# ZJU-FAST-Lab/uneven_planner

Measured on AMD Instinct MI355X. Metric: MINCO traj-opts/sec (batch), higher is better.
Workload: dtype f64

## Files before the change

uneven_planner_amd/csrc/solver_program.hpp:

```cpp
#pragma once
#include "terrain_dev.hpp"
#include "trajectory_dev.hpp"
#include "uph_common.hpp"

namespace uph {

#ifndef UPH_GRID_FROM_MEM
#define UPH_GRID_FROM_MEM 1
#endif
#ifndef UPH_PHASE_MASK
#define UPH_PHASE_MASK 15
#endif
#ifndef UPH_STATE_PROBE
#define UPH_STATE_PROBE(st) do { } while (0)
#endif
#ifndef UPH_SCALING_WB
#define UPH_SCALING_WB 8
#endif
#ifndef UPH_SC_XB
#define UPH_SC_XB 9
#endif
#ifndef UPH_SC_YB
#define UPH_SC_YB 14
#endif
#ifndef UPH_SC_WLO
#define UPH_SC_WLO 2
#endif
#ifndef UPH_SC_WHI
#define UPH_SC_WHI 3
#endif

template <class WG, class SR = double>
struct Solver {
    WG& wg;
    const GridDev& grid;
    const OptParams& P;
    const BatchDev& bd;
    const TrajDesc& td;
    int Nxy, Nyaw, n, S, K, mem, CH, CHP, recd;
    int CHS;
    int* rtag;
    double *x, *xp, *g, *gp, *d, *cxy, *cyaw, *Gxy, *Gyaw, *gamxy, *gamyaw, *bt, *rec, *wtab, *ttab, *pf, *hd;
    double* ab;
    int* abn;
    static constexpr int AB_DOUBLES = 4;
    UPH_HD void tally(int k, bool yes) {
#if defined(__HIP_DEVICE_COMPILE__)
        if (yes && wg.wave == 0) abn[k] = abn[k] + 1;
#else
        if (yes) abn[k]++;
#endif
    }
    double *dual, *res, *scl, *hist;
    int hrow, hnp;
    const double *Wr_xy, *Wr_yaw;
    double rho, scale_fx, Txy, Tyaw, last_jerk, last_gd;
    long long hist_reads;
    long long cyc[16];
    long long t_last_eval_end;
    long long* sub_t = nullptr;
    int evals, bidx, trace_n;
    float inv_k1;
    double ec_irho, ec_step, ec_invK, ec_iTyaw, ec_omega, ec_omega_h;

    static constexpr int REC_FIELDS = 12;
    static UPH_HD size_t ldsDoubles(int Nxy, int Nyaw, int n, int CH, int mem, int K) {
        size_t recd = (size_t)REC_FIELDS * (CH + 1) + (CH + 1) / 2;
        const size_t nvec = 2 * (Nxy + 5) + (Nyaw + 5);
        const size_t knd = (size_t)knotBufDoubles(Nxy + 1, 4) + knotBufDoubles(Nyaw + 1, 2), adj = (size_t)knotBufDoubles(Nxy, 4) + knotBufDoubles(Nyaw, 2) + nvec;
        recd = recd < knd ? knd : recd;
        recd = recd < adj ? adj : recd;
        recd = recd < (size_t)mem ? (size_t)mem : recd;
        const size_t td_ = (size_t)Nxy + K + 2;
        return (size_t)5 * n + (nvec < td_ ? td_ : nvec) + 2 * (12 * Nxy + 6 * Nyaw) + recd + (size_t)6 * (K + 1) + THOMAS_DOUBLES + MAX_PAST + 8 + 18 + AB_DOUBLES;
    }

    UPH_HD Solver(WG& w, const GridDev& gr, const OptParams& p, const BatchDev& b, int bi, double* lds)
        : wg(w), grid(gr), P(p), bd(b), td(b.desc[bi]) {
        bidx = bi;
        Nxy = td.Nxy; Nyaw = td.Nyaw; n = td.n; S = td.S; K = P.int_K; mem = P.mem_size;
        inv_k1 = 1.0f / (float)(K + 1);
        CH = wg.size(); CHP = CH + 1; recd = REC_FIELDS * CHP + (CH + 1) / 2;
        CHS = CH;
#if !defined(UPH_ALIGNED_CHUNKS) || UPH_ALIGNED_CHUNKS
        {
            const int ppc = CH / (K + 1);
            if (ppc >= 1 && (Nxy + ppc - 1) / ppc == (S + CH - 1) / CH) CHS = ppc * (K + 1);
        }
#endif
        double* q = lds;
        x = q; q += n; g = q; q += n; d = q; q += n;
        xp = q; q += n; gp = q; q += n;
        const int nvec = 2 * (Nxy + 5) + (Nyaw + 5);
        bt = q;
        gamxy = q; gamyaw = q + 2 * (Nxy + 5);
        q += nvec < Nxy + K + 2 ? Nxy + K + 2 : nvec;
        cxy = q; q += 12 * Nxy; cyaw = q; q += 6 * Nyaw;
        Gxy = q; q += 12 * Nxy; Gyaw = q; q += 6 * Nyaw;
        wtab = q; q += 6 * (K + 1);
        rec = q;
        {
            size_t rd = (size_t)recd;
            const size_t knd = (size_t)knotBufDoubles(Nxy + 1, 4) + knotBufDoubles(Nyaw + 1, 2), adj = (size_t)knotBufDoubles(Nxy, 4) + knotBufDoubles(Nyaw, 2) + nvec;
            rd = rd < knd ? knd : rd; rd = rd < adj ? adj : rd; rd = rd < (size_t)mem ? (size_t)mem : rd;
            q += rd;
        }
        rtag = (int*)(rec + (size_t)REC_FIELDS * CHP);
        ttab = q; q += THOMAS_DOUBLES;
        pf = q; q += MAX_PAST + 8;
        hd = q; q += 18;
        ab = q; q += AB_DOUBLES;
        abn = (int*)(ab + 1);
        dual = bd.dual + 7 * td.off_s; res = bd.res + 7 * td.off_s; scl = bd.scl + 7 * td.off_s;
        hist = bd.hist + td.off_hist; hrow = histRowDoubles(n); hnp = 64 * histNQ(n);
        Wr_xy = bd.ops[td.op_xy].Wr; Wr_yaw = bd.ops[td.op_yaw].Wr;
        rho = 0; scale_fx = 1.0; Txy = Tyaw = 0; last_jerk = 0; hist_reads = 0; evals = 0; trace_n = 0;
        for (int q = 0; q < 16; q++) cyc[q] = 0;
        t_last_eval_end = 0;
        wg.pfor(18 + THOMAS_DOUBLES, [&](int t) {
            if (t == 0) { ab[0] = 0.0; abn[0] = abn[1] = abn[2] = abn[3] = 0; }
            if (t < 18) hd[t] = t < 6 ? td.init_xy[t] : (t < 12 ? td.end_xy[t - 6] : (t < 15 ? td.init_yaw[t - 12] : td.end_yaw[t - 15]));
            else ttab[t - 18] = bd.thomas[t - 18];
        });
    }

    UPH_HD void tracePush(double v) {
        if (bd.trace != nullptr && trace_n < bd.trace_cap) {
            const int at = trace_n;
            wg.one([&]() { bd.trace[(size_t)bidx * bd.trace_cap + at] = v; });
        }
        trace_n++;
    }

    static UPH_HD int divSmall(int a, int b, float inv) {
        int q = (int)((float)a * inv);
        const int r = a - q * b;
        if (r < 0) q--;
        else if (r >= b) q++;
        return q;
    }
    static UPH_HD int knotCol(int j, int N) { return j == 0 ? 0 : (j == N ? N + 2 : j + 2); }
    UPH_HD double knotPos(const double* xin, int j, int dd) const {
        if (dd < 2) return j == 0 ? hd[dd] : (j == Nxy ? hd[6 + dd] : xin[1 + 2 * (j - 1) + dd]);
        return j == 0 ? hd[12] : (j == Nyaw ? hd[15] : xin[1 + 2 * (Nxy - 1) + (j - 1)]);
    }

    UPH_HD double dot(const double* a, const double* b, int m) {
        double r[1];
        wg.template sum<1>(m, r, [&](int i, double* acc) { acc[0] += a[i] * b[i]; });
        return r[0];
    }
    UPH_HD double absmax(const double* a, int m) {
        return wg.maxv(m, [&](int i) { return fabs(a[i]); });
    }

    template <bool STEP>
    UPH_HD void generate(double* xin, double st) {
        UPH_MARK("generate");
        const long long tsub_start = wg.clock();
        const double tau_ = STEP ? fma(st, d[0], xp[0]) : xin[0];
        const double Ttot = expC2(tau_);
        Txy = wg.bcast(Ttot / (double)Nxy);
        Tyaw = wg.bcast(Ttot / (double)Nyaw);
        ec_iTyaw = wg.bcast(1.0 / Tyaw);
        const double Tx = Txy, Ty = Tyaw;
        double* zxy = rec;
        double* zyaw = rec + knotBufDoubles(Nxy + 1, 4);
        wg.pfor(2 * (Nxy + 1) + (Nyaw + 1), [&](int t) {
            const bool isxy = t < 2 * (Nxy + 1);
            const int j = isxy ? (t >> 1) : t - 2 * (Nxy + 1), dd = isxy ? (t & 1) : 2, N = isxy ? Nxy : Nyaw, os = isxy ? 2 : 1;
            const double T1 = isxy ? Tx : Ty;
            const double* h0 = isxy ? hd + (dd & 1) : hd + 12;
            const double* h1 = isxy ? hd + 6 + (dd & 1) : hd + 15;
            double* z = isxy ? zxy + knotOffJ(j, 4) + (dd & 1) : zyaw + knotOffJ(j, 2);
            if (STEP && t == 0) xin[0] = tau_;
            if (j == 0) { z[0] = T1 * h0[os]; z[os] = T1 * T1 * h0[2 * os]; }
            else if (j == N) { z[0] = T1 * h1[os]; z[os] = T1 * T1 * h1[2 * os]; }
            else {
                double pm, p0, pp;
                if (STEP) {
                    const int ix = isxy ? 1 + 2 * (j - 1) + dd : 1 + 2 * (Nxy - 1) + (j - 1), ws = isxy ? 2 : 1;
                    p0 = fma(st, d[ix], xp[ix]);
                    pm = j == 1 ? h0[0] : fma(st, d[ix - ws], xp[ix - ws]);
                    pp = j == N - 1 ? h1[0] : fma(st, d[ix + ws], xp[ix + ws]);
                    xin[ix] = p0;
                } else { pm = knotPos(xin, j - 1, dd); p0 = knotPos(xin, j, dd); pp = knotPos(xin, j + 1, dd); }
                const double dp = pp - p0, dm = p0 - pm;
                double r0 = 20.0 * (dp - dm), r1 = -15.0 * (dp + dm);
                if (j == 1) { const double v0 = T1 * h0[os], a0 = T1 * T1 * h0[2 * os]; r0 += 8.0 * v0 + a0; r1 += 7.0 * v0 + a0; }
                if (j == N - 1) { const double vN = T1 * h1[os], aN = T1 * T1 * h1[2 * os]; r0 += -8.0 * vN + aN; r1 += 7.0 * vN - aN; }
                z[0] = r0; z[os] = r1;
            }
        });
        const long long tsub1 = wg.clock();
        wg.thomas(ttab, false, zyaw + knotOffJ(1, 2), Nyaw - 1, zxy + knotOffJ(1, 4), Nxy - 1);
        if (sub_t) { sub_t[0] += tsub1 - tsub_start; sub_t[1] += wg.clock() - tsub1; }
    }

    UPH_HD void expand(const double* xin, double jerk_w, double out[3]) {
        UPH_MARK("expand");
        const long long t0 = wg.clock();
        const double Tx = Txy, Ty = Tyaw, itx = wg.bcast(1.0 / Tx), ity = wg.bcast(1.0 / Ty);
        const double* zxy = rec;
        const double* zyaw = rec + knotBufDoubles(Nxy + 1, 4);
        const int np = 2 * Nxy + Nyaw;
        wg.template sum<3>(np + 2, out, [&](int t, double* acc) {
            if (t >= np) { fillTimes(t - np); return; }
            double p0, p1, v0, a0, v1, a1, it_, T1;
            double *oc, *og;
            int os;
            const bool isxy = t < 2 * Nxy;
            if (isxy) {
                const int i = t >> 1, dd = t & 1;
                p0 = knotPos(xin, i, dd); p1 = knotPos(xin, i + 1, dd);
                const double *k0 = zxy + knotOffJ(i, 4) + dd, *k1 = zxy + knotOffJ(i + 1, 4) + dd;
                v0 = k0[0]; a0 = k0[2]; v1 = k1[0]; a1 = k1[2];
                oc = cxy + 12 * i + dd; og = Gxy + 12 * i + dd; os = 2; it_ = itx; T1 = Tx;
            } else {
                const int m = t - 2 * Nxy;
                p0 = knotPos(xin, m, 2); p1 = knotPos(xin, m + 1, 2);
                const double *k0 = zyaw + knotOffJ(m, 2), *k1 = zyaw + knotOffJ(m + 1, 2);
                v0 = k0[0]; a0 = k0[1]; v1 = k1[0]; a1 = k1[1];
                oc = cyaw + 6 * m; og = Gyaw + 6 * m; os = 1; it_ = ity; T1 = Ty;
            }
            const double dl = p1 - p0;
            const double h3 = 10.0 * dl - 6.0 * v0 - 4.0 * v1 - 1.5 * a0 + 0.5 * a1;
            const double h4 = -15.0 * dl + 8.0 * v0 + 7.0 * v1 + 1.5 * a0 - a1;
            const double h5 = 6.0 * dl - 3.0 * v0 - 3.0 * v1 - 0.5 * a0 + 0.5 * a1;
            const double i2 = it_ * it_, i3 = i2 * it_, i4 = i3 * it_, i5 = i4 * it_;
            const double c3 = h3 * i3, c4 = h4 * i4, c5 = h5 * i5;
            oc[0] = p0; oc[os] = v0 * it_; oc[2 * os] = (0.5 * a0) * i2;
            oc[3 * os] = c3; oc[4 * os] = c4; oc[5 * os] = c5;
            const double T2 = T1 * T1, T3 = T2 * T1, T4 = T2 * T2, T5 = T4 * T1;
            og[0] = 0.0; og[os] = 0.0; og[2 * os] = 0.0;
            og[3 * os] = jerk_w * (72.0 * c3 * T1 + 144.0 * c4 * T2 + 240.0 * c5 * T3);
            og[4 * os] = jerk_w * (144.0 * c3 * T2 + 384.0 * c4 * T3 + 720.0 * c5 * T4);
            og[5 * os] = jerk_w * (240.0 * c3 * T3 + 720.0 * c4 * T4 + 1440.0 * c5 * T5);
            const double d33 = c3 * c3, d43 = c4 * c3, d44 = c4 * c4, d53 = c5 * c3, d54 = c5 * c4, d55 = c5 * c5;
            acc[0] += 36.0 * d33 * T1 + 144.0 * d43 * T2 + 192.0 * d44 * T3 + 240.0 * d53 * T3 + 720.0 * d54 * T4 + 720.0 * d55 * T5;
            const double gT = 36.0 * d33 + 288.0 * d43 * T1 + 576.0 * d44 * T2 + 720.0 * d53 * T2 + 2880.0 * d54 * T3 + 3600.0 * d55 * T4;
            acc[1] += isxy ? gT : 0.0;
            acc[2] += isxy ? 0.0 : gT;
        });
        if (sub_t) sub_t[2] += wg.clock() - t0;
    }

    UPH_HD GridDev framedGrid() const {
        if (bd.grid_mem != nullptr && bd.grid_per_traj != 0) return bd.grid_mem[bidx];
        return grid;
    }

    template <class R>
    struct KinT {
        R b0[6], b1[6], b2[6], b3[6];
        R y0[6], y1[6], y2[6];
        R pos[2], vel[2], acc[2], jer[2];
        R yaw, dyaw, d2yaw, cyaw, syaw, v_norm, lon_acc, lat_acc, u, s1;
        R tv[7], tg[7][3];
        R vx, wz, ax, ay, curv_snorm, den, sq;
        R yawn, cw, sw;
        R zx, zy, gs[3], gzx[3], gzy[3];
        int yaw_idx;
    };
    typedef KinT<double> Kin;
    template <class R>
    UPH_HD void terrainValuesOnly(KinT<R>& S_) const {
        R sg;
#if defined(__HIP_DEVICE_COMPILE__) && UPH_GRID_FROM_MEM
        typedef const __attribute__((address_space(4))) unsigned long long* gw_t;
        gw_t T = (gw_t)(const void*)(bd.grid_mem + (size_t)bidx * bd.grid_per_traj);
        asm volatile("" : "+s"(T));
        constexpr int NWORD = (int)(sizeof(GridDev) / 8);
        unsigned long long w[NWORD];
#pragma unroll
        for (int k = 0; k < NWORD; k++) w[k] = T[k];
        GridDev gl;
        __builtin_memcpy(&gl, w, sizeof(GridDev));
        terrainBase<R>(gl, S_.pos[0], S_.pos[1], S_.yawn, sg, S_.zx, S_.zy, S_.gs, S_.gzx, S_.gzy);
#else
        const GridDev gl = framedGrid();
        terrainBase<R>(gl, S_.pos[0], S_.pos[1], S_.yawn, sg, S_.zx, S_.zy, S_.gs, S_.gzx, S_.gzy);
#endif
        const R zx = S_.zx, zy = S_.zy;
        const R cc = sqrt(1.0 - zx * zx - zy * zy);
        const R inv_c = 1.0 / cc;
        const R t = S_.cw * zx + S_.sw * zy;
        const R s = -(-S_.sw * zx + S_.cw * zy);
        const R sq = sqrt(1.0 - t * t);
        const R r = 1.0 / sq;
// ... 268 lines not shown
        const int i0 = s0 / K1, i1 = (s0 + cnt - 1) / K1;
        const int nxyt = 6 * (i1 - i0 + 1);
        const int XYL = (nxyt + 63) & ~63;
        int m0 = rtag[0] - 1, m1 = rtag[cnt - 1] + 1;
        if (m0 < 0) m0 = 0;
        if (m1 > Nyaw - 1) m1 = Nyaw - 1;
        auto xyTask = [&](int t) {
            const int pi = t / 6, r = t - 6 * pi, dd = r & 1, kp = r >> 1;
            const int i = i0 + pi;
            const int ja = i * K1 - s0;
            const int jlo = ja < 0 ? -ja : 0, jhi = cnt - ja < K1 ? cnt - ja : K1;
            const double* r0 = rec + dd * CHP + ja;
            const int k0 = 2 * kp, k1 = k0 + 1;
            const int pa = k0 >= 2 ? k0 - 2 : 0, pb = k0 >= 1 ? k0 - 1 : 0;
            const double c1a = (double)k0, c2a = (double)(k0 * (k0 - 1)), c1b = (double)k1, c2b = (double)(k1 * k0);
            double a0 = 0.0, a1 = 0.0;
            const double* w = wtab;
#pragma unroll 1
            for (int jb = 0; jb < K1; jb += UPH_SC_XB) {
                double e0[UPH_SC_XB], e1[UPH_SC_XB], e2[UPH_SC_XB], pA[UPH_SC_XB], pB[UPH_SC_XB], pC[UPH_SC_XB], pD[UPH_SC_XB];
#pragma unroll
                for (int u = 0; u < UPH_SC_XB; u++) {
                    const int j = jb + u;
                    e0[u] = r0[j]; e1[u] = r0[2 * CHP + j]; e2[u] = r0[4 * CHP + j];
                    pA[u] = w[6 * j + pa]; pB[u] = w[6 * j + pb]; pC[u] = w[6 * j + k0]; pD[u] = w[6 * j + k1];
                }
#pragma unroll
                for (int u = 0; u < UPH_SC_XB; u++) {
                    const int j = jb + u;
                    const bool in = j >= jlo && j < jhi;
                    a0 += in ? (pC[u] * e0[u] + (c1a * pB[u]) * e1[u] + (c2a * pA[u]) * e2[u]) : 0.0;
                    a1 += in ? (pD[u] * e0[u] + (c1b * pC[u]) * e1[u] + (c2b * pB[u]) * e2[u]) : 0.0;
                }
            }
            Gxy[12 * i + 2 * k0 + dd] += a0;
            Gxy[12 * i + 2 * k1 + dd] += a1;
        };
        auto yawTask = [&](int tt) {
            const int mi = tt / 3, kp = tt - 3 * mi, m = m0 + mi;
            const double xa = (double)m * xr, xb = (double)(m + 1) * xr;
            const int pa = (int)xa, pb = (int)xb;
            int sa = pa * K1 + (int)((xa - (double)pa) * (double)K) - UPH_SC_WLO - s0;
            int sb = pb * K1 + (int)((xb - (double)pb) * (double)K) + UPH_SC_WHI - s0;
            if (m == Nyaw - 1) sb = cnt;
            if (sa < 0) sa = 0;
            if (sb > cnt) sb = cnt;
            if (sb < sa) sb = sa;
            const double* rv = rec + (6 + 2 * kp) * CHP + sa;
            const int* tg = rtag + sa;
            double a0 = 0.0, a1 = 0.0;
            for (int len = sb - sa; len > 0; len -= UPH_SC_YB, rv += UPH_SC_YB, tg += UPH_SC_YB) {
                int tg_[UPH_SC_YB];
                double v0[UPH_SC_YB], v1[UPH_SC_YB];
#pragma unroll
                for (int u = 0; u < UPH_SC_YB; u++) { tg_[u] = tg[u]; v0[u] = rv[u]; v1[u] = rv[CHP + u]; }
#pragma unroll
                for (int u = 0; u < UPH_SC_YB; u++) {
                    const bool in = (u < len) && (tg_[u] == m);
                    a0 += in ? v0[u] : 0.0;
                    a1 += in ? v1[u] : 0.0;
                }
            }
            Gyaw[6 * m + 2 * kp] += a0;
            Gyaw[6 * m + 2 * kp + 1] += a1;
        };
        if constexpr (WG::MFMA_SCATTER) {
            if (K1 == 17) {
                UPH_MARK("scatter.mfma");
                wg.scatterXY17(rec, wtab, Gxy, i0, i1 - i0 + 1, s0, cnt);
                UPH_MARK("scatter.yaw");
                wg.pforRev(3 * (m1 - m0 + 1), yawTask);
                return;
            }
        }
        UPH_MARK("scatter.vector(cold for K=16)");
        wg.pfor(XYL + 3 * (m1 - m0 + 1), [&](int t) {
            if (t < XYL) { if (t < nxyt) xyTask(t); }
            else yawTask(t - XYL);
        });
    }

    UPH_HD void adjoint(double& chain_xy, double& chain_yaw, double* gout = nullptr, double* gd_out = nullptr) {
        UPH_MARK("adjoint");
        const double Tx = Txy, Ty = Tyaw, itx = wg.bcast(1.0 / Txy), ity = wg.bcast(1.0 / Tyaw);
        const long long ta0 = wg.clock();
        const int nbx = Nxy + 5, nby = Nyaw + 5;
        const int nvec = 2 * nbx + nby;
        double* gwxy = rec;
        double* gwyaw = gwxy + knotBufDoubles(Nxy, 4);
        double* gdir = gwyaw + knotBufDoubles(Nyaw, 2);
        double ch[2];
        wg.template sum<2>(2 * (Nxy + 1) + (Nyaw + 1), ch, [&](int t, double* acc) {
            const bool isxy = t < 2 * (Nxy + 1);
            const int j = isxy ? (t >> 1) : t - 2 * (Nxy + 1), dd = isxy ? (t & 1) : 0, N = isxy ? Nxy : Nyaw, os = isxy ? 2 : 1;
            const double* G = isxy ? Gxy + dd : Gyaw;
            const double* c = isxy ? cxy + dd : cyaw;
            const double it_ = isxy ? itx : ity;
            const double i2 = it_ * it_, i3 = i2 * it_, i4 = i3 * it_, i5 = i4 * it_;
            double dp = 0.0, dv = 0.0, da = 0.0;
            if (j < N) {
                const double* gl = G + (size_t)6 * j * os;
                const double* cl = c + (size_t)6 * j * os;
                const double r1 = gl[os], r2 = gl[2 * os], r3 = gl[3 * os], r4 = gl[4 * os], r5 = gl[5 * os];
                const double chain = -it_ * (cl[os] * r1 + 2.0 * (cl[2 * os] * r2) + 3.0 * (cl[3 * os] * r3) + 4.0 * (cl[4 * os] * r4) + 5.0 * (cl[5 * os] * r5));
                acc[0] += isxy ? chain : 0.0;
                acc[1] += isxy ? 0.0 : chain;
                const double g0 = gl[0], g1 = r1 * it_, g2 = r2 * i2, g3 = r3 * i3, g4 = r4 * i4, g5 = r5 * i5;
                dp += g0 - 10.0 * g3 + 15.0 * g4 - 6.0 * g5;
                dv += g1 - 6.0 * g3 + 8.0 * g4 - 3.0 * g5;
                da += 0.5 * g2 - 1.5 * g3 + 1.5 * g4 - 0.5 * g5;
            }
            if (j > 0) {
                const double* gr_ = G + (size_t)6 * (j - 1) * os;
                const double g3 = gr_[3 * os] * i3, g4 = gr_[4 * os] * i4, g5 = gr_[5 * os] * i5;
                dp += 10.0 * g3 - 15.0 * g4 + 6.0 * g5;
                dv += -4.0 * g3 + 7.0 * g4 - 3.0 * g5;
                da += 0.5 * g3 - g4 + 0.5 * g5;
            }
            double* gd = isxy ? gdir + dd : gdir + 2 * nbx;
            gd[knotCol(j, N) * os] = dp;
            if (j == 0) { gd[1 * os] = dv; gd[2 * os] = da; }
            else if (j == N) { gd[(N + 3) * os] = dv; gd[(N + 4) * os] = da; }
            else if (isxy) { double* kq = gwxy + knotOff(j - 1, 4) + dd; kq[0] = dv; kq[2] = da; }
            else { double* kq = gwyaw + knotOff(j - 1, 2); kq[0] = dv; kq[1] = da; }
        });
        const long long ta1 = wg.clock();
        wg.thomas(ttab, true, gwyaw, Nyaw - 1, gwxy, Nxy - 1);
        const long long ta2 = wg.clock();
        double hh[3];
        wg.template sum<3>(nvec, hh, [&](int t, double* acc) {
            const bool isxy = t < 2 * nbx;
            const int col = isxy ? (t >> 1) : t - 2 * nbx, dd = isxy ? (t & 1) : 0, N = isxy ? Nxy : Nyaw;
            const int ks = isxy ? 4 : 2, cs = isxy ? 2 : 1;
            const double* lam = isxy ? gwxy + dd : gwyaw;
            const double T1 = isxy ? Tx : Ty;
            const double* h0 = isxy ? hd + dd : hd + 12;
            const double* h1 = isxy ? hd + 6 + dd : hd + 15;
            auto L0 = [&](int j) { return (j >= 1 && j <= N - 1) ? lam[knotOff(j - 1, ks)] : 0.0; };
            auto L1 = [&](int j) { return (j >= 1 && j <= N - 1) ? lam[knotOff(j - 1, ks) + cs] : 0.0; };
            double a = gdir[t], hT = 0.0;
            if (col == 1) { a += 8.0 * L0(1) + 7.0 * L1(1); hT = a * h0[cs]; }
            else if (col == 2) { a += L0(1) + L1(1); hT = a * (2.0 * T1 * h0[2 * cs]); }
            else if (col == N + 3) { a += -8.0 * L0(N - 1) + 7.0 * L1(N - 1); hT = a * h1[cs]; }
            else if (col == N + 4) { a += L0(N - 1) - L1(N - 1); hT = a * (2.0 * T1 * h1[2 * cs]); }
            else {
                const int k = col == 0 ? 0 : (col == N + 2 ? N : col - 2);
                a += 20.0 * ((L0(k - 1) - L0(k)) - (L0(k) - L0(k + 1))) - 15.0 * (L1(k - 1) - L1(k + 1));
            }
            if (isxy) gamxy[t] = a; else gamyaw[t - 2 * nbx] = a;
            acc[0] += isxy ? hT : 0.0;
            acc[1] += isxy ? 0.0 : hT;
            if (gout != nullptr && col >= 3 && col <= N + 1) {
                const int ix = isxy ? 1 + 2 * (col - 3) + dd : 1 + 2 * (Nxy - 1) + (col - 3);
                gout[ix] = a;
                acc[2] += a * d[ix];
            }
        });
        if (gd_out) *gd_out = hh[2];
        if (sub_t) { sub_t[4] += ta1 - ta0; sub_t[5] += ta2 - ta1; sub_t[6] += wg.clock() - ta2; }
        chain_xy = ch[0] + hh[0];
        chain_yaw = ch[1] + hh[1];
    }

    UPH_HD void evalConsts() {
        ec_irho = wg.bcast(1.0 / rho);
        ec_step = wg.bcast(Txy / K);
        ec_invK = wg.bcast(1.0 / K);
        ec_omega = wg.bcast(P.rho_ter * ec_step * scale_fx);
        ec_omega_h = wg.bcast(0.5 * P.rho_ter * ec_step * scale_fx);
    }

    UPH_HD void refreshResiduals() {
        UPH_MARK("refreshResiduals");
        wg.pfor(2, [&](int u) { fillTimes(u); });
        wg.pfor(S, [&](int s) { double dummy[3]; sampleEval<true>(s, 0, dummy); });
    }

    static constexpr double ABANDON_REL = 1e-9, ABANDON_REL_F = 1e-14;
    template <bool STEP>
    UPH_HD double eval(double* xin, double* gout, double st = 0.0, double thr = __builtin_huge_val()) {
        evals++;
        long long t0 = wg.clock();
        if (t_last_eval_end) cyc[5] += t0 - t_last_eval_end;
        if (UPH_PHASE_MASK & 1) generate<STEP>(xin, st);
        const double tau = wg.bcast(xin[0]);
        const double jw = wg.bcast(P.use_scaling ? scale_trick_jerk * scale_fx : scale_fx);
        double js[3] = {0.0, 0.0, 0.0};
        if (UPH_PHASE_MASK & 1) expand(xin, jw, js);
        long long t1 = wg.clock(); cyc[0] += t1 - t0;
        last_jerk = js[0];
        const double jerk_cost = wg.bcast(P.use_scaling ? js[0] * scale_fx * scale_trick_jerk : js[0] * scale_fx);
        evalConsts();
        if (STEP && thr < __builtin_huge_val()) {
            double tq = tau;
            pinv(tq);
            const double tau_lb = P.rho_T * expC2(tq) * scale_fx;
            const double lbd = wg.bcast(ab[0]);
            const double L0 = wg.bcast(jerk_cost + tau_lb - lbd);
            const double mag = wg.bcast(fabs(jerk_cost) + fabs(tau_lb) + lbd);
            if (L0 > thr + ABANDON_REL * mag && L0 < __builtin_huge_val() && ec_omega >= 0.0) {
                tally(2, true);
                t_last_eval_end = wg.clock();
                return L0;
            }
        }
        double sm[3] = {0.0, 0.0, 0.0};
        wg.template accBegin<3>();
        for (int s0 = 0; s0 < S; s0 += CHS) {
            const int cnt = S - s0 < CHS ? S - s0 : CHS;
            t0 = wg.clock();
            if (UPH_PHASE_MASK & 2) wg.template accChunk<3>(cnt, [&](int t, double* acc) { sampleEval<false, SR>(s0 + t, t, acc); });
            t1 = wg.clock(); cyc[1] += t1 - t0;
            if (UPH_PHASE_MASK & 4) scatterChunk(s0, cnt);
            cyc[2] += wg.clock() - t1;
        }
        wg.template accEnd<3>(sm);
        t1 = wg.clock();
        if (STEP && thr < __builtin_huge_val()) {
            double tq = tau;
            pinv(tq);
            const double tau_q = P.rho_T * expC2(tq) * scale_fx;
            const double fq = wg.bcast(jerk_cost + sm[0] + tau_q);
            const double mag = wg.bcast(fabs(jerk_cost) + fabs(sm[0]) + fabs(tau_q));
            if (fq > thr + ABANDON_REL_F * mag && fq < __builtin_huge_val()) {
                tally(3, true);
                t_last_eval_end = wg.clock();
                return fq;
            }
        }
        double chx = 0.0, chy = 0.0, gdw = 0.0;
        if (UPH_PHASE_MASK & 8) adjoint(chx, chy, gout, &gdw);
        t0 = wg.clock(); cyc[3] += t0 - t1;
        const double gTx = js[1] * jw + sm[1] + chx;
        const double gTy = js[2] * jw + sm[2] + chy;
        const double grad_Tsum = P.rho_T * scale_fx + gTx / Nxy + gTy / Nyaw;
        const double g0 = wg.bcast(grad_Tsum * getTtoTauGrad(tau));
        wg.pfor(1, [&](int) { gout[0] = g0; });
        last_gd = wg.bcast(gdw + g0 * d[0]);
        const double tau_cost = P.rho_T * expC2(tau) * scale_fx;
        t_last_eval_end = wg.clock();
        return wg.bcast(jerk_cost + sm[0] + tau_cost);
    }

    UPH_HD void initScaling(double* x0) {
        generate<false>(x0, 0.0);
        const double tau = x0[0];
        const double dTau = getTtoTauGrad(tau);
        double js[3];
        expand(x0, 1.0, js);
        double sm[3] = {0.0, 0.0, 0.0};
        for (int s0 = 0; s0 < S; s0 += CHS) {
            const int cnt = S - s0 < CHS ? S - s0 : CHS;
            double part[3];
            wg.template sum<3>(cnt, part, [&](int t, double* acc) { sampleObjective(s0 + t, t, acc); });
            sm[0] += part[0]; sm[1] += part[1]; sm[2] += part[2];
            scatterChunk(s0, cnt);
        }
        double chx, chy;
        adjoint(chx, chy);
        const double gTau_fx = (P.rho_T + (js[1] + sm[1] + chx) / Nxy + (js[2] + sm[2] + chy) / Nyaw) * dTau;
        const double mq = wg.maxv((Nxy - 1) * 2 + (Nyaw - 1), [&](int t) {
            return t < (Nxy - 1) * 2 ? fabs(gamxy[3 * 2 + t]) : fabs(gamyaw[3 + (t - (Nxy - 1) * 2)]);
        });
        scale_fx = wg.bcast(1.0 / dmax(1.0, dmax(mq, fabs(gTau_fx))));
        wg.pfor(2, [&](int u) { fillTimes(u); });
        wg.pfor(S, [&](int s) { scalingSample(s, dTau); });
    }

    UPH_HD void scalingSample(int s, double dTau) {
        const int i = divSmall(s, K + 1, inv_k1), j = s - i * (K + 1);
        Kin k;
        kin(i, j, k);
#if !defined(UPH_SCALING_GROUPS) || UPH_SCALING_GROUPS == 2
        scalingGroup<0, 4>(s, i, j, k, dTau);
        scalingGroup<4, 3>(s, i, j, k, dTau);
#elif UPH_SCALING_GROUPS == 3
        scalingGroup<0, 3>(s, i, j, k, dTau);
        scalingGroup<3, 2>(s, i, j, k, dTau);
        scalingGroup<5, 2>(s, i, j, k, dTau);
#else
        scalingGroup<0, 7>(s, i, j, k, dTau);
#endif
    }
    template <int Q0, int NQS>
    UPH_HD void scalingGroup(int s, int i, int j, const Kin& k, double dTau) {
        const int nbx = Nxy + 5, nby = Nyaw + 5;
        const double Tx = Txy, Ty = Tyaw, itx = 1.0 / Txy, ity = 1.0 / Tyaw;
        const double gravity = grid.gravity;
        const double alpha = 1.0 / K * j;
        const double icvx = k.tv[0], icvy = k.tv[2], icxi = k.tv[5];
        const int m = k.yaw_idx;
        double dpL[NQS][2], dvL[NQS][2], daL[NQS][2], dpR[NQS][2], dvR[NQS][2], daR[NQS][2];
        double ypL[NQS], yvL[NQS], yaL[NQS], ypR[NQS], yvR[NQS], yaR[NQS];
        double sumx[NQS], sumy[NQS], mx[NQS];
#pragma unroll
        for (int qi = 0; qi < NQS; qi++) {
            const int q = Q0 + qi;
            double gp_[2] = {0, 0}, gv_[2] = {0, 0}, ga_[2] = {0, 0}, gyaw = 0.0, gdyaw = 0.0, gse2[3];
            if (q == 0) {
                gv_[0] = k.syaw; gv_[1] = -k.cyaw;
                gyaw = k.vel[0] * k.cyaw + k.vel[1] * k.syaw;
            } else if (q == 1) {
                for (int t = 0; t < 2; t++) gv_[t] = 1.0 * icvx * icvx * 2.0 * k.vel[t];
                for (int t = 0; t < 3; t++) gse2[t] = 1.0 * k.v_norm * k.v_norm * 2.0 * icvx * k.tg[0][t];
                gp_[0] = gse2[0]; gp_[1] = gse2[1]; gyaw = gse2[2];
            } else if (q == 2) {
                const double gax = 2.0 * k.ax;
                ga_[0] = gax * icvx * k.cyaw; ga_[1] = gax * icvx * k.syaw;
                gyaw = gax * icvx * k.lat_acc;
                for (int t = 0; t < 3; t++) gse2[t] = gax * (gravity * k.tg[1][t] + k.tg[0][t] * k.lon_acc);
                gp_[0] = gse2[0]; gp_[1] = gse2[1]; gyaw += gse2[2];
            } else if (q == 3) {
                const double gay = 2.0 * k.ay;
                ga_[0] = gay * icvy * (-k.syaw); ga_[1] = gay * icvy * k.cyaw;
                gyaw = -gay * icvy * k.lon_acc;
                for (int t = 0; t < 3; t++) gse2[t] = gay * (gravity * k.tg[3][t] + k.tg[2][t] * k.lat_acc);
                gp_[0] = gse2[0]; gp_[1] = gse2[1]; gyaw += gse2[2];
            } else if (q == 4) {
                const double den = 1.0 / (k.vx * k.vx + delta_sigl);
                const double gwz = den * 2.0 * k.wz;
                const double gvx2 = -k.curv_snorm * den;
                gdyaw = gwz * icxi;
// ... 366 lines not shown
        });
        const long long tstart = wg.clock();
        if (P.use_scaling) initScaling(x);
        cyc[5] += wg.clock() - tstart;
        wg.pfor(1, [&](int) { st.scale_fx = scale_fx; st.cyc[5] = cyc[5]; });
    }

    UPH_HD void optimize(TrajState& st, int cap = 0) {
        double* gx0 = bd.x + td.off_x;
        rho = wg.bcast(st.rho);
        scale_fx = wg.bcast(st.scale_fx);
        wg.pfor(n, [&](int t) { x[t] = gx0[t]; });
        formDualBound();
        const long long tstart = wg.clock();
        cyc[14] = wg.realtime();
        int ret_code = 0, iter = 0, total_k = 0, last_ret = 0;
        double inner_cost = 0.0;
        while (true) {
            int kk = 0;
            tracePush(-1.0);
            const int result = lbfgs<false>(inner_cost, kk);
            refreshResiduals();
            total_k += kk;
            last_ret = result;
            if (result == LBFGS_CONVERGENCE || result == LBFGS_CANCELED || result == LBFGS_STOP || result == LBFGSERR_MAXIMUMITERATION) {
            } else if (result == LBFGSERR_MAXIMUMLINESEARCH) {
            } else { ret_code = 1; break; }
            updateDualVars();
            if (judgeConvergence()) break;
            if (++iter > P.max_iter) { ret_code = 2; break; }
            if (cap > 0 && iter >= cap) { ret_code = 3; break; }
        }
        wg.pfor(n, [&](int t) { gx0[t] = x[t]; bd.gout[td.off_x + t] = g[t]; });
        cyc[6] = wg.clock() - tstart;
        cyc[15] = wg.realtime();
        storeTrajectory(st);
        wg.pfor(1, [&](int) {
            st.ret_code = ret_code; st.alm_iters = iter; st.lbfgs_iters = total_k; st.last_lbfgs_ret = last_ret; st.f = inner_cost;
        });
    }

    UPH_HD void resumeHook(TrajState& st, int budget, int finish) {
        double* gx = bd.x + td.off_x;
        double* gg = bd.gout + td.off_x;
        double* gd = bd.rs_d + td.off_x;
        double* rs = bd.rs + (size_t)bidx * 24;
        rho = wg.bcast(st.rho); scale_fx = wg.bcast(st.scale_fx);
        formDualBound();
        wg.pfor(n + MAX_PAST, [&](int t) { if (t < n) { x[t] = gx[t]; g[t] = gg[t]; d[t] = gd[t]; } else pf[t - n] = rs[8 + t - n]; });
        ResumeIO io;
        io.step = wg.bcast(rs[0]); io.fx = wg.bcast(rs[1]);
        io.k = (int)wg.bcast(rs[2]); io.end = (int)wg.bcast(rs[3]); io.bound = (int)wg.bcast(rs[4]); io.budget = budget;
        double f = 0.0;
        int kk = 0;
        const int ret = lbfgs<true>(f, kk, &io);
        int accepted = 0, conv = 0;
        if (evals > 0) refreshResiduals();
        if (finish && ret != LBFGS_RUNNING_HOOK) {
            accepted = (ret == LBFGS_CONVERGENCE || ret == LBFGS_CANCELED || ret == LBFGS_STOP || ret == LBFGSERR_MAXIMUMITERATION || ret == LBFGSERR_MAXIMUMLINESEARCH) ? 1 : 0;
            if (accepted) { updateDualVars(); conv = judgeConvergence() ? 1 : 0; }
        }
        wg.pfor(n + MAX_PAST, [&](int t) { if (t < n) { gx[t] = x[t]; gg[t] = g[t]; gd[t] = d[t]; } else rs[8 + t - n] = pf[t - n]; });
        wg.pfor(1, [&](int) {
            rs[0] = io.step; rs[1] = io.fx; rs[2] = io.k; rs[3] = io.end; rs[4] = io.bound; rs[5] = ret; rs[6] = accepted; rs[7] = conv;
            st.f = io.fx; st.last_lbfgs_ret = ret; st.lbfgs_iters = io.k;
        });
        storeTrajectory(st);
    }

    UPH_HD void microbench(TrajState& st, int reps) {
        const double* gx0 = bd.x + td.off_x;
        rho = wg.bcast(st.rho); scale_fx = wg.bcast(st.scale_fx);
        wg.pfor(n, [&](int t) { x[t] = gx0[t]; d[t] = 0.5; xp[t] = gx0[t]; gp[t] = 0.25; });
        long long a[9];
        long long sub[8] = {0, 0, 0, 0, 0, 0, 0, 0};
        sub_t = sub;
        double acc = 0.0, js[3], part[3], c1, c2;
        const int cnt = S < CH ? S : CH;
        a[0] = wg.clock();
        for (int r = 0; r < reps; r++) generate<false>(x, 0.0);
        a[1] = wg.clock();
        for (int r = 0; r < reps; r++) { expand(x, 1.0, js); acc += js[0]; }
        a[2] = wg.clock();
        for (int r = 0; r < reps; r++) evalConsts();
        a[3] = wg.clock();
        for (int r = 0; r < reps; r++) { wg.template sum<3>(cnt, part, [&](int t, double* ac) { sampleEval<false>(t, t, ac); }); acc += part[0]; }
        a[4] = wg.clock();
        for (int r = 0; r < reps; r++) scatterChunk(0, cnt);
        a[5] = wg.clock();
        for (int r = 0; r < reps; r++) { adjoint(c1, c2); acc += c1 + c2; }
        a[6] = wg.clock();
        const int m = mem;
        for (int r = 0; r < reps; r++) {
            const int end = (r * 7) % m, bound = m;
            acc += absmax(g, n) + absmax(x, n);
            wg.sync();
            wg.pfor(1, [&](int) { pf[r % 3] = acc; });
            double* sc = hist + (size_t)end * hrow + 2;
            double* yc = sc + hnp;
            double r6[6] = {0, 0, 0, 0, 0, 0};
            wg.template sum<3>(n, r6, [&](int i, double* ac) {
                const double sv = x[i] - xp[i], yv = g[i] - gp[i];
                sc[i] = sv; yc[i] = yv;
                ac[0] += yv * sv; ac[1] += yv * yv; ac[2] += sv * sv;
                d[i] = -g[i];
            });
            acc += r6[0] + r6[3] + sqrt(dot(gp, gp, n));
            wg.sync();
            wg.pfor(1, [&](int) { hist[(size_t)end * hrow] = acc; });
            (void)bound;
        }
        a[7] = wg.clock();
        wg.pfor(1, [&](int) {
            for (int q = 0; q < 7; q++) st.cyc[q] = (a[q + 1] - a[q]) / reps;
            st.cyc[7] = a[7] - a[0];
            for (int q = 0; q < 8; q++) st.cyc[8 + q] = sub[q] / reps;
            st.f = acc;
        });
        sub_t = nullptr;
    }

    UPH_HD void evalOnly(TrajState& st, int repeat) {
        const double* gx0 = bd.x + td.off_x;
        rho = wg.bcast(st.rho); scale_fx = wg.bcast(st.scale_fx);
        wg.pfor(n, [&](int t) { x[t] = gx0[t]; });
        double f = 0.0;
        for (int r = 0; r < repeat; r++) f = eval<false>(x, g);
        refreshResiduals();
        wg.pfor(n, [&](int t) { bd.gout[td.off_x + t] = g[t]; });
        storeTrajectory(st);
        wg.pfor(1, [&](int) { st.f = f; });
    }
    template <bool STORE_RES>
    UPH_HD void penaltyOnly(TrajState& st, int repeat) {
        rho = wg.bcast(st.rho); scale_fx = wg.bcast(st.scale_fx);
        Txy = wg.bcast(st.T_xy); Tyaw = wg.bcast(st.T_yaw);
        ec_iTyaw = wg.bcast(1.0 / Tyaw);
        const double* oc = bd.cxy + td.off_cxy;
        const double* oy = bd.cyaw + td.off_cyaw;
        const int nc = 12 * Nxy + 6 * Nyaw;
        wg.pfor(nc, [&](int t) { if (t < 12 * Nxy) cxy[t] = oc[t]; else cyaw[t - 12 * Nxy] = oy[t - 12 * Nxy]; });
        double sm[3] = {0.0, 0.0, 0.0};
        for (int r = 0; r < repeat; r++) {
            wg.pfor(nc + 2, [&](int t) { if (t < 12 * Nxy) Gxy[t] = 0.0; else if (t < nc) Gyaw[t - 12 * Nxy] = 0.0; else fillTimes(t - nc); });
            evalConsts();
            wg.template accBegin<3>();
            for (int s0 = 0; s0 < S; s0 += CHS) {
                const int cnt = S - s0 < CHS ? S - s0 : CHS;
                wg.template accChunk<3>(cnt, [&](int t, double* acc) { sampleEval<STORE_RES ? 2 : 0, SR>(s0 + t, t, acc); });
                scatterChunk(s0, cnt);
            }
            wg.template accEnd<3>(sm);
        }
        double* ogx = bd.pen_gxy + td.off_cxy;
        double* ogy = bd.pen_gyaw + td.off_cyaw;
        wg.pfor(nc + 1, [&](int t) {
            if (t < 12 * Nxy) ogx[t] = Gxy[t];
            else if (t < nc) ogy[t - 12 * Nxy] = Gyaw[t - 12 * Nxy];
            else { double* o = bd.pen_out + (size_t)bidx * 3; o[0] = sm[0]; o[1] = sm[1]; o[2] = sm[2]; }
        });
    }
    UPH_HD void scalingOnly(TrajState& st) {
        const double* gx0 = bd.x + td.off_x;
        rho = wg.bcast(st.rho); scale_fx = 1.0;
        wg.pfor(n, [&](int t) { x[t] = gx0[t]; });
        initScaling(x);
        storeTrajectory(st);
    }

    UPH_HD void report(const TrajState& st) {
        const double* oc = bd.cxy + td.off_cxy;
        const double* oy = bd.cyaw + td.off_cyaw;
        wg.pfor(12 * Nxy + 6 * Nyaw, [&](int t) { if (t < 12 * Nxy) cxy[t] = oc[t]; else cyaw[t - 12 * Nxy] = oy[t - 12 * Nxy]; });
        const double Tx = st.T_xy, Ty = st.T_yaw;
        double durx = 0.0, dury = 0.0;
        for (int i = 0; i < Nxy; i++) durx += Tx;
        for (int i = 0; i < Nyaw; i++) dury += Ty;
        const double total = dmin(durx, dury);
        int cnt = 0;
        {
            double cnt_d[1];
            wg.template sum<1>(1, cnt_d, [&](int, double* acc) { double t = 0.0; int q = 0; for (; q < 200000 && t < total; q++) t += 0.01; acc[0] += (double)q; });
            cnt = (int)cnt_d[0];
        }
        const double gravity = grid.gravity;
        const GridDev fgrid = framedGrid();
        double tcur = 0.0;
        int qcur = 0;
        auto sampleAt = [&](int q, double out[7]) {
            if (q < qcur) { tcur = 0.0; qcur = 0; }
            for (; qcur < q; qcur++) tcur += 0.01;
            TrajSample smp;
            trajectorySample<true>(cxy, cyaw, Nxy, Nyaw, Tx, Ty, tcur, fgrid, gravity, smp, out);
        };
        double o[7], e1[1], ma[7], mb[3], dum[1];
        wg.template sumMax<1, 7>(cnt, e1, ma, [&](int q, double* acc, double* mx) {
            double r[7];
            sampleAt(q, r);
            acc[0] += r[6];
            mx[0] = dmax(mx[0], r[0]); mx[1] = dmax(mx[1], -r[0]); mx[2] = dmax(mx[2], r[1]); mx[3] = dmax(mx[3], -r[1]);
            mx[4] = dmax(mx[4], r[2]); mx[5] = dmax(mx[5], -r[2]); mx[6] = dmax(mx[6], r[3]);
        });
        wg.template sumMax<1, 3>(cnt, dum, mb, [&](int q, double* acc, double* mx) {
            double r[7];
            sampleAt(q, r);
            acc[0] += 0.0;
            mx[0] = dmax(mx[0], -r[3]); mx[1] = dmax(mx[1], r[4] + 1.0); mx[2] = dmax(mx[2], r[5]);
        });
        o[0] = ma[0] >= ma[1] ? ma[0] : -ma[1];
        o[1] = ma[2] >= ma[3] ? ma[2] : -ma[3];
        o[2] = ma[4] >= ma[5] ? ma[4] : -ma[5];
        o[3] = ma[6] >= mb[0] ? ma[6] : -mb[0];
        o[4] = mb[1] - 1.0;
        o[5] = mb[2];
        o[6] = e1[0];
        wg.pfor(7, [&](int t) { bd.report[(size_t)bidx * 7 + t] = o[t]; });
    }
};

}
```

uneven_planner_amd/csrc/unevenhip.hip:

```cpp
#include <hip/hip_runtime.h>

#include <type_traits>

#include <algorithm>
#include <cmath>
#include <cstdio>
#include <cstdlib>
#include <cstring>
#include <map>
#include <numeric>
#include <string>
#include <thread>
#include <vector>

#include "../../include/uneven_hip.h"
#include "minco_op_host.hpp"
#include "resample_walk.hpp"
#include "solver_program.hpp"
#include "uph_ctx.hpp"
#include "wave_dev.hpp"

using namespace uph;

#ifndef UPH_THOMAS_KPL
// ... 345 lines not shown
            const int j = j0 + k;
            const bool v = j <= len;
            const double r0 = v ? pk[k * ks] : 0.0, r1 = v ? pk[k * ks + cs] : 0.0;
            double P[4], M1[4];
            thomasFactors<ADJ>(tab, v ? j : 1, P, M1, Qm[k], M2[k]);
#pragma unroll
            for (int q = 0; q < 4; q++) { if (!v) { P[q] = 0.0; M1[q] = 0.0; Qm[k][q] = 0.0; M2[k][q] = 0.0; } }
            double t0, t1;
            mv2(P, r0, r1, t0, t1);
            if (k == 0) {
                c[0][0] = t0; c[0][1] = t1;
#pragma unroll
                for (int q = 0; q < 4; q++) F[0][q] = -M1[q];
            } else {
                submv2(t0, t1, M1, c[k - 1][0], c[k - 1][1], c[k][0], c[k][1]);
                F[k][0] = -fma(M1[1], F[k - 1][2], M1[0] * F[k - 1][0]); F[k][1] = -fma(M1[1], F[k - 1][3], M1[0] * F[k - 1][1]);
                F[k][2] = -fma(M1[3], F[k - 1][2], M1[2] * F[k - 1][0]); F[k][3] = -fma(M1[3], F[k - 1][3], M1[2] * F[k - 1][1]);
            }
        }
        const int steps = (lmax + KPL - 1) / KPL;
        double y0 = 0.0, y1 = 0.0;
        for (int s = 0; s < steps; s++) {
            const double p0 = shr1(y0), p1 = shr1(y1);
            y0 = fma(F[KPL - 1][1], p1, fma(F[KPL - 1][0], p0, c[KPL - 1][0]));
            y1 = fma(F[KPL - 1][3], p1, fma(F[KPL - 1][2], p0, c[KPL - 1][1]));
        }
        double yk[KPL][2];
        {
            const double p0 = shr1(y0), p1 = shr1(y1);
#pragma unroll
            for (int k = 0; k < KPL; k++) {
                yk[k][0] = fma(F[k][1], p1, fma(F[k][0], p0, c[k][0]));
                yk[k][1] = fma(F[k][3], p1, fma(F[k][2], p0, c[k][1]));
            }
        }
#pragma unroll
        for (int k = KPL - 1; k >= 0; k--) {
            double t0, t1;
            mv2(Qm[k], yk[k][0], yk[k][1], t0, t1);
            if (k == KPL - 1) {
                c[k][0] = t0; c[k][1] = t1;
#pragma unroll
                for (int q = 0; q < 4; q++) F[k][q] = -M2[k][q];
            } else {
                submv2(t0, t1, M2[k], c[k + 1][0], c[k + 1][1], c[k][0], c[k][1]);
                F[k][0] = -fma(M2[k][1], F[k + 1][2], M2[k][0] * F[k + 1][0]); F[k][1] = -fma(M2[k][1], F[k + 1][3], M2[k][0] * F[k + 1][1]);
                F[k][2] = -fma(M2[k][3], F[k + 1][2], M2[k][2] * F[k + 1][0]); F[k][3] = -fma(M2[k][3], F[k + 1][3], M2[k][2] * F[k + 1][1]);
            }
        }
        double z0 = 0.0, z1 = 0.0;
        for (int s = 0; s < steps; s++) {
            const double p0 = shl1(z0), p1 = shl1(z1);
            z0 = fma(F[0][1], p1, fma(F[0][0], p0, c[0][0]));
            z1 = fma(F[0][3], p1, fma(F[0][2], p0, c[0][1]));
        }
        {
            const double p0 = shl1(z0), p1 = shl1(z1);
#pragma unroll
            for (int k = 0; k < KPL; k++) {
                if (j0 + k <= len) {
                    pk[k * ks] = fma(F[k][1], p1, fma(F[k][0], p0, c[k][0]));
                    pk[k * ks + cs] = fma(F[k][3], p1, fma(F[k][2], p0, c[k][1]));
                }
            }
        }
    }
    template <bool ADJ>
    __device__ __forceinline__ void thomasT(const double* tab, double* bw, int lenW, double* bx, int lenX) {
        UPH_MARK("thomas");
        __builtin_amdgcn_s_setprio(3);
        const bool packed = uni(lenW) <= 32 * UPH_THOMAS_KPL - 1 && uni(lenX) <= 16 * UPH_THOMAS_KPL - 1;
        if (packed) {
            if (wave == 0) thomasWave<2, ADJ, UPH_THOMAS_KPL>(tab, bw, lenW, bx, lenX);
        } else if (NW >= 2) {
            if (wave == 0) thomasWave<0, ADJ, UPH_THOMAS_KPL>(tab, bw, lenW, bx, lenX);
            else if (wave == 1) thomasWave<1, ADJ, UPH_THOMAS_KPL>(tab, bw, lenW, bx, lenX);
        } else {
            thomasWave<0, ADJ, UPH_THOMAS_KPL>(tab, bw, lenW, bx, lenX);
            thomasWave<1, ADJ, UPH_THOMAS_KPL>(tab, bw, lenW, bx, lenX);
        }
        __builtin_amdgcn_s_setprio(0);
        bar(2);
    }
    __device__ __forceinline__ void thomas(const double* tab, bool adj, double* bw, int lenW, double* bx, int lenX) {
        if (adj) thomasT<true>(tab, bw, lenW, bx, lenX);
        else thomasT<false>(tab, bw, lenW, bx, lenX);
    }
    __device__ __forceinline__ void twoLoop(double* d, const double* g, int n, const double* __restrict__ hist, double* dg_out, double* al_lds, int m, int end, int bound, double scale) {
        if (wave == 0) {
            __builtin_amdgcn_s_setprio(3);
            constexpr int PF = UPH_TWOLOOP_PF;
            const int nq = uni((n + 63) >> 6);
            if (nq == 1) twoLoopT<1, PF>(d, g, dg_out, al_lds, n, hist, m, end, bound, scale);
            else if (nq == 2) twoLoopT<2, PF>(d, g, dg_out, al_lds, n, hist, m, end, bound, scale);
            else if (nq == 3) twoLoopT<3, PF>(d, g, dg_out, al_lds, n, hist, m, end, bound, scale);
            else if (nq == 4) twoLoopT<4, PF>(d, g, dg_out, al_lds, n, hist, m, end, bound, scale);
            else if (nq == 5) twoLoopT<5, 2>(d, g, dg_out, al_lds, n, hist, m, end, bound, scale);
            else if (nq == 6) twoLoopT<6, 2>(d, g, dg_out, al_lds, n, hist, m, end, bound, scale);
            else if (nq == 7) twoLoopT<7, 2>(d, g, dg_out, al_lds, n, hist, m, end, bound, scale);
            else twoLoopT<8, 2>(d, g, dg_out, al_lds, n, hist, m, end, bound, scale);
            __builtin_amdgcn_s_setprio(0);
        }
        bar(1);
    }
    template <class F>
    __device__ __forceinline__ double maxv(int n, F f) {
        double a = 0.0;
        for (int i = ftid(); i < n; i += NT) { const double v = f(i); a = v > a ? v : a; }
        a = waveMax(a);
        double* r = red + par * (NW * MAXM);
        par ^= 1;
        if (lane == 0) r[wave * MAXM] = a;
        bar(0);
        double t = r[0];
#pragma unroll
        for (int w = 1; w < NW; w++) t = r[w * MAXM] > t ? r[w * MAXM] : t;
        return uni(t);
    }
};

template <int NT, int WPS, int MODE, bool F32S = false>
__global__ __launch_bounds__(NT, WPS) void uph_solver_kernel(GridDev grid, OptParams P, BatchDev bd, int repeat) {
    extern __shared__ double lds[];
    const int w = blockIdx.x;
    if (w >= bd.B) return;
    const int b = bd.order ? bd.order[w] : w;
    DevWG<NT> wg(lds);
    typedef typename std::conditional<F32S, f32r, double>::type SR;
    Solver<DevWG<NT>, SR> sol(wg, grid, P, bd, b, lds + DevWG<NT>::SCRATCH);
    TrajState& st = bd.state[b];
    if (MODE == 0) sol.evalOnly(st, repeat);
    else if (MODE == 1) sol.prepare(st);
    else if (MODE == 2) sol.optimize(st, repeat);
    else if (MODE == 7) sol.resumeHook(st, repeat >> 1, repeat & 1);
    else if (MODE == 8) { if (repeat & 1) sol.template penaltyOnly<true>(st, repeat >> 1); else sol.template penaltyOnly<false>(st, repeat >> 1); }
    else if (MODE == 3) sol.report(st);
    else if (MODE == 5) sol.microbench(st, repeat);
    else sol.scalingOnly(st);
}

__global__ void uph_fill_kernel(double* __restrict__ p, size_t n, double v) {
    for (size_t i = (size_t)blockIdx.x * blockDim.x + threadIdx.x; i < n; i += (size_t)gridDim.x * blockDim.x) p[i] = v;
}

__global__ void uph_terrain_kernel(GridDev grid, const double* __restrict__ pos, int n, double* __restrict__ values, double* __restrict__ grads) {
    const int i = blockIdx.x * blockDim.x + threadIdx.x;
    if (i >= n) return;
    const double yaw = pos[3 * i + 2];
    double v[7], g[7][3];
    terrainAllWithGrad(grid, pos[3 * i], pos[3 * i + 1], yaw, cos(yaw), sin(yaw), v, g);
    for (int k = 0; k < 7; k++) {
        values[7 * i + k] = v[k];
        for (int q = 0; q < 3; q++) grads[21 * i + 3 * k + q] = g[k][q];
    }
}

constexpr int PLAN_SX = UPH_MAX_PIECE_XY - 1, PLAN_SY = UPH_MAX_PIECE_YAW - 1;
struct PlanHead {
    int32_t n_inner_xy, n_inner_yaw;
    int32_t short_path, pad;
    double p_init[2], p_end[2];
    double yaw_init, yaw_end;
    double total_time;
    double lo[2], hi[2];
    double turn, kink;
};
struct PlanPath {
    const double* p;
    __host__ __device__ double operator()(int64_t k, int j) const { return p[3 * k + j]; }
};
struct PlanSink {
    double *oxy, *oyw;
    int nxy, nyw;
    double nlo[2], nhi[2], prev, turn, kink;
    __device__ void xy(double x, double y) {
        if (nxy < PLAN_SX) { oxy[2 * nxy] = x; oxy[2 * nxy + 1] = y; }
        nxy++;
        nlo[0] = x < nlo[0] ? x : nlo[0]; nlo[1] = y < nlo[1] ? y : nlo[1];
        nhi[0] = nhi[0] < x ? x : nhi[0]; nhi[1] = nhi[1] < y ? y : nhi[1];
    }
    __device__ void yaw(double v) {
        if (nyw < PLAN_SY) oyw[nyw] = v;
        nyw++;
        const double d = fabs(v - prev);
        turn += d; kink = kink < d ? d : kink; prev = v;
    }
    __device__ void unwrapped(int64_t, double) {}
};
__global__ __launch_bounds__(64) void uph_plan_resample_kernel(uph_manager_params mp, const double* __restrict__ paths, int path_cap, const int* __restrict__ n_path,
                                                               const int* __restrict__ status, int nq, const int* __restrict__ goal_of, double* __restrict__ st_xy,
                                                               double* __restrict__ st_yaw, PlanHead* __restrict__ heads) {
#pragma clang fp contract(off)
    const int q = blockIdx.x * blockDim.x + threadIdx.x;
    if (q >= nq) return;
    const int m = n_path[q];
    if (status[q] != UPH_KINO_OK || m > path_cap) return;
    const int g = goal_of ? goal_of[q] : q;
    PlanHead h = PlanHead{};
    if (m < 2) { h.short_path = 1; heads[g] = h; return; }
    const double* p = paths + (size_t)q * path_cap * 3;
    const WalkSetup ws = walkSetup(mp);
    PlanSink s;
// ... 1306 lines not shown
```

Before: 53110.

## Overlap per-eval constant prep and time tables with the Thomas knot solve

Adds an 'aside' helper that runs a small task on an otherwise idle wave while the wave(s) running the Thomas solve work. That task computes the inverse durations, the sample step, exp(tau) and its tau gradient, and fills the time tables. Expand, adjoint and eval then read these cached values from LDS instead of recomputing divisions and exp per call, and expand no longer needs its extra fillTimes tasks. This relies on the aside wave's LDS writes being visible after the Thomas barrier. Choosing the wave is heuristic, and with a single wave the aside work runs serially.

```diff
diff --git a/uneven_planner_amd/csrc/solver_program.hpp b/uneven_planner_amd/csrc/solver_program.hpp
--- a/uneven_planner_amd/csrc/solver_program.hpp
+++ b/uneven_planner_amd/csrc/solver_program.hpp
@@ -29,6 +29,15 @@
 #ifndef UPH_SC_WHI
 #define UPH_SC_WHI 3
 #endif
+
+#ifndef UPH_ASIDE_PREP
+#define UPH_ASIDE_PREP 1
+#endif
+template <class WG, class F>
+UPH_HD void asideKnotSolve(WG& wg, int lenW, int lenX, int n, F f) {
+    (void)lenW; (void)lenX;
+    wg.pfor(n, f);
+}
 
 template <class WG, class SR = double>
 struct Solver {
@@ -44,6 +53,8 @@
     double* ab;
     int* abn;
     static constexpr int AB_DOUBLES = 4;
+    double* up;
+    static constexpr int UP_DOUBLES = 6;
     UPH_HD void tally(int k, bool yes) {
 #if defined(__HIP_DEVICE_COMPILE__)
         if (yes && wg.wave == 0) abn[k] = abn[k] + 1;
@@ -72,7 +83,7 @@
         recd = recd < adj ? adj : recd;
         recd = recd < (size_t)mem ? (size_t)mem : recd;
         const size_t td_ = (size_t)Nxy + K + 2;
-        return (size_t)5 * n + (nvec < td_ ? td_ : nvec) + 2 * (12 * Nxy + 6 * Nyaw) + recd + (size_t)6 * (K + 1) + THOMAS_DOUBLES + MAX_PAST + 8 + 18 + AB_DOUBLES;
+        return (size_t)5 * n + (nvec < td_ ? td_ : nvec) + 2 * (12 * Nxy + 6 * Nyaw) + recd + (size_t)6 * (K + 1) + THOMAS_DOUBLES + MAX_PAST + 8 + 18 + AB_DOUBLES + UP_DOUBLES;
     }
 
     UPH_HD Solver(WG& w, const GridDev& gr, const OptParams& p, const BatchDev& b, int bi, double* lds)
@@ -111,6 +122,7 @@
         hd = q; q += 18;
         ab = q; q += AB_DOUBLES;
         abn = (int*)(ab + 1);
+        up = q; q += UP_DOUBLES;
         dual = bd.dual + 7 * td.off_s; res = bd.res + 7 * td.off_s; scl = bd.scl + 7 * td.off_s;
         hist = bd.hist + td.off_hist; hrow = histRowDoubles(n); hnp = 64 * histNQ(n);
         Wr_xy = bd.ops[td.op_xy].Wr; Wr_yaw = bd.ops[td.op_yaw].Wr;
@@ -162,7 +174,9 @@
         const double Ttot = expC2(tau_);
         Txy = wg.bcast(Ttot / (double)Nxy);
         Tyaw = wg.bcast(Ttot / (double)Nyaw);
+#if !(UPH_ASIDE_PREP)
         ec_iTyaw = wg.bcast(1.0 / Tyaw);
+#endif
         const double Tx = Txy, Ty = Tyaw;
         double* zxy = rec;
         double* zyaw = rec + knotBufDoubles(Nxy + 1, 4);
@@ -193,18 +207,40 @@
             }
         });
         const long long tsub1 = wg.clock();
+#if UPH_ASIDE_PREP
+        asideKnotSolve(wg, Nyaw - 1, Nxy - 1, 2, [&](int t) {
+            const double itx = 1.0 / Tx, ity = 1.0 / Ty, step = Tx / K, dtau = getTtoTauGrad(tau_);
+            if (t == 0) { up[0] = itx; up[1] = ity; up[2] = step; up[3] = Ttot; up[4] = dtau; }
+            const double add = t == 0 ? Tx : step;
+            double* tab = t == 0 ? bt : bt + Nxy + 1;
+            const int lim = t == 0 ? Nxy : K, top = Nxy > K ? Nxy : K;
+            double a = 0.0;
+            for (int i = 0; i <= top; i++) {
+                if (i <= lim) tab[i] = a;
+                a += add;
+            }
+        });
+#endif
         wg.thomas(ttab, false, zyaw + knotOffJ(1, 2), Nyaw - 1, zxy + knotOffJ(1, 4), Nxy - 1);
+#if UPH_ASIDE_PREP
+        ec_iTyaw = wg.bcast(up[1]);
+#endif
         if (sub_t) { sub_t[0] += tsub1 - tsub_start; sub_t[1] += wg.clock() - tsub1; }
     }
 
     UPH_HD void expand(const double* xin, double jerk_w, double out[3]) {
         UPH_MARK("expand");
         const long long t0 = wg.clock();
+#if UPH_ASIDE_PREP
+        const double Tx = Txy, Ty = Tyaw, itx = wg.bcast(up[0]), ity = ec_iTyaw;
+        const int np = 2 * Nxy + Nyaw, ntask = np;
+#else
         const double Tx = Txy, Ty = Tyaw, itx = wg.bcast(1.0 / Tx), ity = wg.bcast(1.0 / Ty);
+        const int np = 2 * Nxy + Nyaw, ntask = np + 2;
+#endif
         const double* zxy = rec;
         const double* zyaw = rec + knotBufDoubles(Nxy + 1, 4);
-        const int np = 2 * Nxy + Nyaw;
-        wg.template sum<3>(np + 2, out, [&](int t, double* acc) {
+        wg.template sum<3>(ntask, out, [&](int t, double* acc) {
             if (t >= np) { fillTimes(t - np); return; }
             double p0, p1, v0, a0, v1, a1, it_, T1;
             double *oc, *og;
@@ -639,7 +675,11 @@
 
     UPH_HD void adjoint(double& chain_xy, double& chain_yaw, double* gout = nullptr, double* gd_out = nullptr) {
         UPH_MARK("adjoint");
+#if UPH_ASIDE_PREP
+        const double Tx = Txy, Ty = Tyaw, itx = wg.bcast(up[0]), ity = ec_iTyaw;
+#else
         const double Tx = Txy, Ty = Tyaw, itx = wg.bcast(1.0 / Txy), ity = wg.bcast(1.0 / Tyaw);
+#endif
         const long long ta0 = wg.clock();
         const int nbx = Nxy + 5, nby = Nyaw + 5;
         const int nvec = 2 * nbx + nby;
@@ -719,9 +759,16 @@
         chain_yaw = ch[1] + hh[1];
     }
 
-    UPH_HD void evalConsts() {
+    UPH_HD double evalStep() {
+#if UPH_ASIDE_PREP
+        return wg.bcast(up[2]);
+#else
+        return Txy / K;
+#endif
+    }
+    UPH_HD void evalConsts(double step) {
         ec_irho = wg.bcast(1.0 / rho);
-        ec_step = wg.bcast(Txy / K);
+        ec_step = wg.bcast(step);
         ec_invK = wg.bcast(1.0 / K);
         ec_omega = wg.bcast(P.rho_ter * ec_step * scale_fx);
         ec_omega_h = wg.bcast(0.5 * P.rho_ter * ec_step * scale_fx);
@@ -747,11 +794,17 @@
         long long t1 = wg.clock(); cyc[0] += t1 - t0;
         last_jerk = js[0];
         const double jerk_cost = wg.bcast(P.use_scaling ? js[0] * scale_fx * scale_trick_jerk : js[0] * scale_fx);
-        evalConsts();
+        evalConsts(evalStep());
         if (STEP && thr < __builtin_huge_val()) {
+#if UPH_ASIDE_PREP
+            double eq = wg.bcast(up[3]);
+            pinv(eq);
+            const double tau_lb = P.rho_T * eq * scale_fx;
+#else
             double tq = tau;
             pinv(tq);
             const double tau_lb = P.rho_T * expC2(tq) * scale_fx;
+#endif
             const double lbd = wg.bcast(ab[0]);
             const double L0 = wg.bcast(jerk_cost + tau_lb - lbd);
             const double mag = wg.bcast(fabs(jerk_cost) + fabs(tau_lb) + lbd);
@@ -774,9 +827,15 @@
         wg.template accEnd<3>(sm);
         t1 = wg.clock();
         if (STEP && thr < __builtin_huge_val()) {
+#if UPH_ASIDE_PREP
+            double eq = wg.bcast(up[3]);
+            pinv(eq);
+            const double tau_q = P.rho_T * eq * scale_fx;
+#else
             double tq = tau;
             pinv(tq);
             const double tau_q = P.rho_T * expC2(tq) * scale_fx;
+#endif
             const double fq = wg.bcast(jerk_cost + sm[0] + tau_q);
             const double mag = wg.bcast(fabs(jerk_cost) + fabs(sm[0]) + fabs(tau_q));
             if (fq > thr + ABANDON_REL_F * mag && fq < __builtin_huge_val()) {
@@ -791,10 +850,16 @@
         const double gTx = js[1] * jw + sm[1] + chx;
         const double gTy = js[2] * jw + sm[2] + chy;
         const double grad_Tsum = P.rho_T * scale_fx + gTx / Nxy + gTy / Nyaw;
+#if UPH_ASIDE_PREP
+        const double g0 = wg.bcast(grad_Tsum * wg.bcast(up[4]));
+        const double etau = wg.bcast(up[3]);
+#else
         const double g0 = wg.bcast(grad_Tsum * getTtoTauGrad(tau));
+        const double etau = expC2(tau);
+#endif
         wg.pfor(1, [&](int) { gout[0] = g0; });
         last_gd = wg.bcast(gdw + g0 * d[0]);
-        const double tau_cost = P.rho_T * expC2(tau) * scale_fx;
+        const double tau_cost = P.rho_T * etau * scale_fx;
         t_last_eval_end = wg.clock();
         return wg.bcast(jerk_cost + sm[0] + tau_cost);
     }
@@ -1327,7 +1392,7 @@
         a[1] = wg.clock();
         for (int r = 0; r < reps; r++) { expand(x, 1.0, js); acc += js[0]; }
         a[2] = wg.clock();
-        for (int r = 0; r < reps; r++) evalConsts();
+        for (int r = 0; r < reps; r++) evalConsts(evalStep());
         a[3] = wg.clock();
         for (int r = 0; r < reps; r++) { wg.template sum<3>(cnt, part, [&](int t, double* ac) { sampleEval<false>(t, t, ac); }); acc += part[0]; }
         a[4] = wg.clock();
@@ -1388,7 +1453,7 @@
         double sm[3] = {0.0, 0.0, 0.0};
         for (int r = 0; r < repeat; r++) {
             wg.pfor(nc + 2, [&](int t) { if (t < 12 * Nxy) Gxy[t] = 0.0; else if (t < nc) Gyaw[t - 12 * Nxy] = 0.0; else fillTimes(t - nc); });
-            evalConsts();
+            evalConsts(Txy / K);
             wg.template accBegin<3>();
             for (int s0 = 0; s0 < S; s0 += CHS) {
                 const int cnt = S - s0 < CHS ? S - s0 : CHS;
diff --git a/uneven_planner_amd/csrc/unevenhip.hip b/uneven_planner_amd/csrc/unevenhip.hip
--- a/uneven_planner_amd/csrc/unevenhip.hip
+++ b/uneven_planner_amd/csrc/unevenhip.hip
@@ -451,6 +451,15 @@
         __builtin_amdgcn_s_setprio(0);
         bar(2);
     }
+    template <class F>
+    __device__ __forceinline__ void aside(int lenW, int lenX, int n, F f) {
+        const bool packed = uni(lenW) <= 32 * UPH_THOMAS_KPL - 1 && uni(lenX) <= 16 * UPH_THOMAS_KPL - 1;
+        const int aw = NW >= 2 && packed ? 1 : (NW >= 3 ? 2 : 0);
+        if (wave == aw) {
+            const int l = flane();
+            if (l < n) f(l);
+        }
+    }
     __device__ __forceinline__ void thomas(const double* tab, bool adj, double* bw, int lenW, double* bx, int lenX) {
         if (adj) thomasT<true>(tab, bw, lenW, bx, lenX);
         else thomasT<false>(tab, bw, lenW, bx, lenX);
@@ -487,6 +496,9 @@
         return uni(t);
     }
 };
+
+template <int NT, class F>
+__device__ __forceinline__ void asideKnotSolve(DevWG<NT>& wg, int lenW, int lenX, int n, F f) { wg.aside(lenW, lenX, n, f); }
 
 template <int NT, int WPS, int MODE, bool F32S = false>
 __global__ __launch_bounds__(NT, WPS) void uph_solver_kernel(GridDev grid, OptParams P, BatchDev bd, int repeat) {
```

Measured after the change: 54200, median of 6. +2.1%, better.
